# chayanchatterjee/GW-Whisper

Measured on AMD Instinct MI355X. Metric: 1s-strain segments/sec (encoder fwd), higher is better.
Workload: dtype bf16; 1 GPU; whisper-tiny encoder fwd, batch 256 log-mel (80x3000) per GPU, 1500 tokens, random-init weights (BASELINE configs[1]); global_batch=256, parallelism=dp1, encoder=tiny, streams_per_gpu=1

## Files before the change

### gw_whisper_amd/csrc/mlp_fused.hip

```cpp
#include "common.h"

#include <stdlib.h>

#include <type_traits>

namespace gww {

namespace {
constexpr int MF_D = 384;
constexpr int MF_KT = MF_D / 64;
constexpr int MF_OT = MF_D / 32;
constexpr int MF_WAVES = 4, MF_THREADS = 256, MF_BM = 128;
#ifndef GWW_MF_EXP
#define GWW_MF_EXP 0
#endif
#ifndef GWW_MF_ABL
#define GWW_MF_ABL 0
#endif
#ifndef GWW_MF_OLDDMA
#define GWW_MF_OLDDMA 0
#endif
#ifndef GWW_MF_AHEAD
#define GWW_MF_AHEAD 3
#endif
// ... 13 lines not shown
#define MF_NT " nt"
#else
#define MF_NT ""
#endif
#ifndef GWW_MF_PADNOP
#define GWW_MF_PADNOP 0
#endif
#if GWW_MF_PADNOP
#define MF_PADNOP "s_nop 1\n\t"
#else
#define MF_PADNOP ""
#endif
#ifndef GWW_MF_XLDS
#define GWW_MF_XLDS 0
#endif
#ifndef GWW_MF_XSTNT
#define GWW_MF_XSTNT 0
#endif
#ifndef GWW_MF_XNT
#define GWW_MF_XNT 0
#endif
#if GWW_MF_XNT
#define MF_XNT MF_NT
#else
#define MF_XNT ""
#endif
#ifndef GWW_MF_XN_LDNT
#define GWW_MF_XN_LDNT 1
#endif
#ifndef GWW_MF_XN_STNT
#define GWW_MF_XN_STNT 1
#endif
#if GWW_MF_XN_LDNT
#define MF_XN_LDNT " nt"
#else
#define MF_XN_LDNT ""
#endif
#if GWW_MF_XN_STNT
#define MF_XN_STNT " nt"
#else
#define MF_XN_STNT ""
#endif
#ifndef GWW_MF_DMAGAP
#define GWW_MF_DMAGAP 1
#endif
#ifndef GWW_MF_TAIL2
#define GWW_MF_TAIL2 0
#endif
#ifndef GWW_MF_NORM
#define GWW_MF_NORM 1
#endif
#ifndef GWW_MF_XACC
#define GWW_MF_XACC 1
#endif
constexpr int MF_AHEAD = GWW_MF_AHEAD;
constexpr int MF_NST_MAX = MF_AHEAD + 1;
constexpr int MF_TILE = 128 * 64 * 2;
constexpr int MF_GL = 16 / MF_WAVES;
constexpr int MF_FMAX = 1536;
constexpr int MF_SLICE_STRIDE = 144, MF_SLICE_BYTES = 32 * MF_SLICE_STRIDE;
constexpr int MF_OFF_CB = MF_NST_MAX * MF_TILE;
constexpr int MF_OFF_U = MF_OFF_CB + MF_FMAX * 4;
constexpr int MF_OFF_B2 = MF_OFF_U + MF_FMAX * 4;
constexpr int MF_OFF_BO = MF_OFF_B2 + MF_D * 4;
constexpr int MF_OFF_QCB = MF_OFF_BO + MF_D * 4;
constexpr int MF_OFF_SLICE = MF_OFF_QCB + MF_FMAX * 4;
constexpr int MF_LDS = MF_OFF_SLICE + 2 * MF_WAVES * MF_SLICE_BYTES;
static_assert(MF_LDS <= 160 * 1024, "LDS budget");

template <int N>
using MF_FL = std::integral_constant<int, N>;

__device__ __forceinline__ float mf_sum8(float v) {
  v += __builtin_bit_cast(float, __builtin_amdgcn_update_dpp(0, __builtin_bit_cast(int, v), 0xB1, 0xF, 0xF, true));
  v += __builtin_bit_cast(float, __builtin_amdgcn_update_dpp(0, __builtin_bit_cast(int, v), 0x4E, 0xF, 0xF, true));
  v += __builtin_bit_cast(float, __builtin_amdgcn_update_dpp(0, __builtin_bit_cast(int, v), 0x141, 0xF, 0xF, true));
  return v;
}

template <int N>
__device__ __forceinline__ void mf_wait_vmcnt() {
  asm volatile("s_waitcnt vmcnt(%0)" ::"n"(N) : "memory");
}

__device__ __forceinline__ float gelu_sig(float x) {
  const float s = fminf(x * x, 64.0f);
  float q = fmaf(s, 0.0010148164f, -0.1067791331f);
  q = fmaf(s, q, -2.3011178f);
#if GWW_MF_EXP & 32
  const float e = (x * q) * 0.37f;
  return x * ((1.0f + e) * 0.91f);
#else
  const float e = __builtin_amdgcn_exp2f(x * q);
  return x * __builtin_amdgcn_rcpf(1.0f + e);
#endif
}

#ifdef GWW_STAMP
__device__ unsigned long long g_stamp_mlp[24];
#define MSTAMP_DECL unsigned long long _t0 = __builtin_amdgcn_s_memtime(); unsigned long long _acc[20] = {0}; \
  const unsigned long long _tb = _t0, _rb = __builtin_amdgcn_s_memrealtime();
#define MSTAMP(i)                                                  \
  do {                                                             \
    if (GWW_STAMP >= 2 && (i) != 0 && (i) != 3 && (i) != 4 && (i) != 5 && !((i) >= 100)) break; \
    __builtin_amdgcn_sched_barrier(0);                             \
    const unsigned long long _t1 = __builtin_amdgcn_s_memtime();   \
    _acc[(i) >= 100 ? (i) - 100 : (i)] += _t1 - _t0;               \
    _t0 = _t1;                                                     \
    __builtin_amdgcn_sched_barrier(0);                             \
  } while (0)
#define TSTAMP(i) do { if (GWW_STAMP == 3) MSTAMP(100 + (i)); } while (0)
#define MSTAMP_FLUSH                                                                 \
  if (lane == 0) {                                                                   \
    for (int _q = 0; _q < 20; ++_q) atomicAdd(&g_stamp_mlp[_q], _acc[_q]);           \
    atomicAdd(&g_stamp_mlp[21], __builtin_amdgcn_s_memrealtime() - _rb);             \
    atomicAdd(&g_stamp_mlp[22], __builtin_amdgcn_s_memtime() - _tb);                 \
    atomicAdd(&g_stamp_mlp[23], 1ull);                                                \
  }
#else
#define MSTAMP_DECL
#define MSTAMP(i)
#define TSTAMP(i)
#define MSTAMP_FLUSH
#endif
}

__device__ __forceinline__ const float* mf_x0_row(const MfX0& z, const float* X, long g, bool x0, bool& tail, int& seg) {
  tail = false; seg = 0;
  if (!x0) return X + g * MF_D;
  const unsigned b = (unsigned)g / (unsigned)z.T, j = (unsigned)g - b * (unsigned)z.T;
  seg = (int)b;
  tail = (int)j >= z.Tt - 2 && (int)j <= z.T - 2;
  if (tail) return z.pos + (long)j * MF_D;
  return z.xs + ((long)b * z.Tt + ((int)j == z.T - 1 ? z.Tt - 1 : (int)j)) * MF_D;
}

struct MfNoX0 {};
template <int MODE, bool OP, bool X0 = false, int XL = 0>
__global__ __launch_bounds__(MF_THREADS, 1) void k_mlp_fused(const float* X, const unsigned short* delta, float* x_out,
                                                            const float* __restrict__ ln_u,
                                                            const float* __restrict__ ln_cb,
                                                            const unsigned short* __restrict__ Wt,
                                                            const float* __restrict__ b2,
                                                            unsigned short* __restrict__ C, long M, int F,
                                                            int stagger_ticks, const float* __restrict__ q_u,
                                                            const float* __restrict__ q_cb,
                                                            unsigned short* __restrict__ q_out, int NQ,
                                                            float* x_next, const float* __restrict__ bo, int keep_x_new,
                                                            const std::conditional_t<X0, MfX0, MfNoX0> z) {
  __shared__ __attribute__((aligned(16))) unsigned char lds[MF_LDS];
  constexpr bool QKV = MODE == 1 || MODE == 2, LNQ = MODE == 2, FIN = MODE == 3;
  static_assert(!X0 || (GWW_MF_NORM && GWW_MF_XACC && (MODE == 2 || (MODE == 1 && OP))), "X0: layer 0's two launches; stages in the u table");
  constexpr bool XACC = GWW_MF_XACC && GWW_MF_NORM && GWW_MF_SCHED && OP && (MODE == 1 || MODE == 3);
  constexpr bool XIN = (XL & 1) != 0, XOUT = (XL & 2) != 0;
  static_assert(XL == 0 || (XACC && !GWW_MF_XLDS && !X0 && (!XOUT || MODE == 1) && XL <= 3), "XL: the accumulator-order stream of XACC");
  constexpr int MF_NST = MF_AHEAD + 1;
  float* lds_cb = reinterpret_cast<float*>(lds + MF_OFF_CB);
  float* lds_u = reinterpret_cast<float*>(lds + MF_OFF_U);
  float* lds_b2 = reinterpret_cast<float*>(lds + MF_OFF_B2);
  float* lds_bo = reinterpret_cast<float*>(lds + MF_OFF_BO);
  float* lds_qcb = reinterpret_cast<float*>(lds + MF_OFF_QCB);
  constexpr int OP_TILES = OP ? 3 * MF_KT : 0;
  typedef __attribute__((address_space(3))) void* lds_ptr;

  const int tid = threadIdx.x, lane = tid & 63, wave = tid >> 6;
  const int r = lane & 31, hh = lane >> 5;
  const long m_base = (long)blockIdx.x * MF_BM + wave * 32;
  unsigned char* slice = lds + MF_OFF_SLICE + wave * MF_SLICE_BYTES;
  unsigned char* const slice0 = slice;
  const int crow = lane >> 3, cchunk = lane & 7;

  const int wave_u = __builtin_amdgcn_readfirstlane(wave);
  const unsigned lane_off = (unsigned)lane * 16u;
  const unsigned lds_base = (unsigned)(unsigned long long)(lds_ptr)lds;
  auto issue_piece_c = [&](int tile, int stage, auto j_c) {
    constexpr int J = decltype(j_c)::value;
    const unsigned dst = lds_base + (unsigned)(stage * MF_TILE + MF_GL * wave_u * 1024);
    if (GWW_MF_EXP & 8) tile &= 7;
    const unsigned short* src = Wt + ((long)tile * (MF_TILE / 2) + MF_GL * wave_u * 512);
    const unsigned lo = lane_off;
    asm volatile("s_mov_b32 m0, %2\n\ts_nop 0\n\tglobal_load_lds_dwordx4 %0, %1 offset:%3"
                 :
                 : "v"(lo), "s"(src), "s"(dst), "n"(J * 1024)
                 : "memory");
  };
  auto issue_piece = [&](int tile, int stage, int j) {
#if GWW_MF_OLDDMA
    const unsigned dst = lds_base + (unsigned)(stage * MF_TILE + (MF_GL * wave_u + j) * 1024);
    const unsigned short* src = Wt + ((long)tile * (MF_TILE / 2) + (MF_GL * wave_u + j) * 512);
    unsigned keep;
    asm volatile("s_mov_b32 %0, m0\n\ts_mov_b32 m0, %3\n\ts_nop 0\n\tglobal_load_lds_dwordx4 %1, %2\n\ts_mov_b32 m0, %0"
                 : "=&s"(keep) : "v"(lane_off), "s"(src), "s"(dst) : "memory");
#else
    if (j == 0) issue_piece_c(tile, stage, std::integral_constant<int, 0>{});
    else if (j == 1) issue_piece_c(tile, stage, std::integral_constant<int, 1>{});
    else if (j == 2) issue_piece_c(tile, stage, std::integral_constant<int, 2>{});
    else issue_piece_c(tile, stage, std::integral_constant<int, 3>{});
#endif
  };
  auto issue = [&](int tile, int stage) {
#pragma unroll
    for (int j = 0; j < MF_GL; ++j) issue_piece(tile, stage, j);
  };

  MSTAMP_DECL
  auto stage_tables = [&]() {
    for (int i = tid; i < F; i += MF_THREADS) {
      lds_cb[i] = GWW_MF_SCHED ? ln_cb[i] * 0.125f : ln_cb[i];
      if (!GWW_MF_NORM) lds_u[i] = ln_u[i];
    }
    if (!GWW_MF_NORM && FIN) __syncthreads();
    if (!LNQ)
      for (int i = tid; i < MF_D; i += MF_THREADS) lds_b2[i] = XACC ? b2[i] + bo[i] : b2[i];
    if (OP)
      for (int i = tid; i < MF_D; i += MF_THREADS) lds_bo[i] = bo[i];
    if (FIN)
      for (int i = tid; i < MF_D; i += MF_THREADS) { lds_u[i] = q_u[i]; lds_u[MF_D + i] = q_cb[i]; }
    if (QKV && GWW_MF_NORM)
      for (int i = tid; i < NQ; i += MF_THREADS) lds_qcb[i] = q_cb[i];
  };
  if constexpr (!XACC) stage_tables();
  if (stagger_ticks > 0 && blockIdx.x < 256) {
    const unsigned long long t0 = __builtin_amdgcn_s_memrealtime();
    const unsigned long long wait = (unsigned long long)((blockIdx.x >> 3) & 15) * stagger_ticks;
    while (__builtin_amdgcn_s_memrealtime() - t0 < wait) __builtin_amdgcn_s_sleep(8);
  }

#pragma unroll
  for (int p = 0; p < MF_AHEAD; ++p) issue(p, p);
  const long xrow_l = m_base + r < M ? m_base + r : M - 1;
  const unsigned xoff = (unsigned)xrow_l * (unsigned)(MF_D * 4) + 16u * (unsigned)hh;
  const unsigned xoff_n = (unsigned)(xrow_l >> 5) * (unsigned)(32 * MF_D * 4) + 16u * (((unsigned)xrow_l & 31u) + 32u * (unsigned)hh);
  f32x4 xp[XACC ? MF_OT : 1][4];
  bool x0 = false;
  int x0_seg0 = 0;
  f32x4* const lds_x0 = reinterpret_cast<f32x4*>(lds + MF_OFF_U);
  const float* x0_stage[2] = {nullptr, nullptr};
  f32x4 x0_sg[2];
  bool x0_tail = false;
  int x0_seg = 0;
  if constexpr (X0) {
    x0 = __builtin_amdgcn_readfirstlane(*z.flag) != 0;
    const unsigned g0 = (unsigned)blockIdx.x * (unsigned)MF_BM;
    x0_seg0 = (int)(g0 / (unsigned)z.T);
    const int seg_last = (int)((unsigned)(M - 1) / (unsigned)z.T);
#pragma unroll
    for (int k = 0; k < 2; ++k) {
      const int q = tid + 256 * k < 4 * (MF_D / 4) ? tid + 256 * k : tid;
      const int sg = q / (2 * (MF_D / 4)), wh = (q / (MF_D / 4)) & 1, c = q % (MF_D / 4);
      const long b = x0_seg0 + sg < seg_last ? x0_seg0 + sg : seg_last;
      x0_stage[k] = (wh ? z.tr + b * MF_D : z.xs + (b * z.Tt + (z.Tt - 2)) * MF_D) + 4 * c;
    }
  }
  auto x0_publish = [&](f32x4 (&sg)[2]) {
    lds_x0[tid] = sg[0];
    if (tid + 256 < 4 * (MF_D / 4)) lds_x0[tid + 256] = sg[1];
    asm volatile("s_waitcnt lgkmcnt(0)" ::: "memory");
    __builtin_amdgcn_s_barrier();
    asm volatile("" ::: "memory");
  };
  if constexpr (XACC && X0) {
    const float* xsrc = mf_x0_row(z, X, xrow_l, x0, x0_tail, x0_seg) + 4 * hh;
#pragma unroll
    for (int t = 0; t < MF_OT; ++t)
#pragma unroll
      for (int cc = 0; cc < 4; ++cc)
        asm volatile("global_load_dwordx4 %0, %1, off offset:%2" MF_XNT : "=a"(xp[t][cc]) : "v"(xsrc), "n"((32 * t + 8 * cc) * 4) : "memory");
#pragma unroll
    for (int k = 0; k < 2; ++k) asm volatile("global_load_dwordx4 %0, %1, off" : "=v"(x0_sg[k]) : "v"(x0_stage[k]) : "memory");
  } else if constexpr (XACC) {
#pragma unroll
    for (int t = 0; t < MF_OT; ++t)
#pragma unroll
      for (int cc = 0; cc < 4; ++cc)
        if (GWW_MF_ABL & 32) asm volatile("v_accvgpr_write_b32 %0, 0" : "=a"(xp[t][cc][0]));
        else if constexpr (XIN)
          asm volatile("global_load_dwordx4 %0, %1, %2 offset:%3" MF_XN_LDNT : "=a"(xp[t][cc]) : "v"(xoff_n), "s"(reinterpret_cast<const char*>(X) + 4096 * t), "n"(1024 * cc) : "memory");
        else asm volatile("global_load_dwordx4 %0, %1, %2 offset:%3" MF_XNT : "=a"(xp[t][cc]) : "v"(xoff), "s"(X), "n"((32 * t + 8 * cc) * 4) : "memory");
  }
  bf16x8 af[MF_KT * 4];
  float row_rstd, row_mean;
  long grow[4];
#pragma unroll
  for (int i = 0; i < 4; ++i) {
    const long g = m_base + 8 * i + crow;
    grow[i] = g < M ? g : M - 1;
  }
  if constexpr (XACC) {
    const unsigned coff = (unsigned)xrow_l * (unsigned)(MF_D * 2) + 64u * (unsigned)hh;
#pragma unroll
    for (int S = 0; S < MF_KT; ++S)
#pragma unroll
      for (int j = 0; j < 4; ++j)
        asm volatile("global_load_dwordx4 %0, %1, %2 offset:%3" : "=v"(af[4 * S + j]) : "v"(coff), "s"(delta), "n"((64 * S + 8 * j) * 2) : "memory");
    if constexpr (X0) {
      if (x0) {
        asm volatile("s_waitcnt vmcnt(24)" : "+v"(x0_sg[0]), "+v"(x0_sg[1]) : : "memory");
#pragma unroll
        for (int t = 0; t < MF_OT; ++t) asm volatile("" : "+a"(xp[t][0]), "+a"(xp[t][1]), "+a"(xp[t][2]), "+a"(xp[t][3]));
        x0_publish(x0_sg);
        if (x0_tail) {
          const f32x4* const st = lds_x0 + (x0_seg - x0_seg0) * (2 * (MF_D / 4)) + hh;
#pragma unroll
          for (int t = 0; t < MF_OT; ++t)
#pragma unroll
            for (int cc = 0; cc < 4; ++cc) {
              const f32x4 xt = st[8 * t + 2 * cc], rt = st[MF_D / 4 + 8 * t + 2 * cc];
#pragma unroll
              for (int k = 0; k < 4; ++k) xp[t][cc][k] = __builtin_fmaf(xt[k], rt[k], xp[t][cc][k]);
            }
        }
      }
    }
    stage_tables();
    asm volatile("s_waitcnt vmcnt(0)" ::: "memory");
#pragma unroll
    for (int i = 0; i < MF_KT * 4; ++i) asm volatile("" : "+v"(af[i]));
    row_rstd = 1.f; row_mean = 0.f;
  } else if constexpr (OP) {
    const unsigned short* crow_p[4];
#pragma unroll
    for (int i = 0; i < 4; ++i) crow_p[i] = delta + grow[i] * MF_D + 8 * cchunk;
    u32x4 cv[MF_KT][4];
#pragma unroll
    for (int S = 0; S < MF_KT; ++S)
#pragma unroll
      for (int i = 0; i < 4; ++i) {
        if (GWW_MF_ABL & 64) { cv[S][i] = u32x4{0x3f803f80u, 0x3f803f80u, 0x3f803f80u, 0x3f803f80u}; continue; }
        asm volatile("global_load_dwordx4 %0, %1, off offset:%2" MF_NT : "=v"(cv[S][i]) : "v"(crow_p[i]), "n"(64 * S * 2) : "memory");
      }
#pragma unroll
    for (int S = 0; S < MF_KT; ++S) {
#pragma unroll
      for (int i = 0; i < 4; ++i) {
        if (!(GWW_MF_ABL & 64)) asm volatile("s_waitcnt vmcnt(%1)" : "+v"(cv[S][i]) : "n"(23 - (4 * S + i)));
        *reinterpret_cast<u32x4*>(slice + (8 * i + crow) * MF_SLICE_STRIDE + cchunk * 16) = cv[S][i];
      }
#pragma unroll
      for (int j = 0; j < 4; ++j) {
        u32x4 u = *reinterpret_cast<const u32x4*>(slice + r * MF_SLICE_STRIDE + (4 * hh + j) * 16);
        asm volatile("" : "+v"(u)::"memory");
        af[4 * S + j] = __builtin_bit_cast(bf16x8, u);
      }
    }
    row_rstd = 1.f; row_mean = 0.f;
  } else
  {
    float s1[4] = {0.f, 0.f, 0.f, 0.f}, s2[4] = {0.f, 0.f, 0.f, 0.f}, cshift[4];
    const float* xrow[4];
    const unsigned short* drow[4];
#pragma unroll
    for (int i = 0; i < 4; ++i) {
      xrow[i] = X + grow[i] * MF_D + 4 * cchunk;
      drow[i] = LNQ ? nullptr : delta + grow[i] * MF_D + 4 * cchunk;
    }
    bool tl[4] = {false, false, false, false};
    const f32x4* st_row[4] = {lds_x0, lds_x0, lds_x0, lds_x0};
    if constexpr (X0) {
#pragma unroll
      for (int i = 0; i < 4; ++i) {
        int seg;
        xrow[i] = mf_x0_row(z, X, grow[i], x0, tl[i], seg) + 4 * cchunk;
        st_row[i] = lds_x0 + (seg - x0_seg0) * (2 * (MF_D / 4)) + cchunk;
      }
#pragma unroll
      for (int k = 0; k < 2; ++k) asm volatile("global_load_dwordx4 %0, %1, off" : "=v"(x0_sg[k]) : "v"(x0_stage[k]) : "memory");
    }
#pragma unroll
    for (int S3 = 0; S3 < MF_KT; S3 += 3) {
      f32x4 xv[3][2][4];
// ... 63 lines not shown
        for (int j = 0; j < 4; ++j) {
          u32x4 u = *reinterpret_cast<const u32x4*>(slice + r * MF_SLICE_STRIDE + (4 * hh + j) * 16);
          asm volatile("" : "+v"(u)::"memory");
          af[4 * S + j] = __builtin_bit_cast(bf16x8, u);
        }
      }
    }
    TSTAMP(8);
    float* stat = reinterpret_cast<float*>(slice);
#pragma unroll
    for (int i = 0; i < 4; ++i) {
      float a = s1[i], b = s2[i];
      a = mf_sum8(a); b = mf_sum8(b);
      const float mean = a * (1.0f / MF_D);
      const float var = fmaxf(b * (1.0f / MF_D) - mean * mean, 0.f);
      if (cchunk == 0) {
        stat[8 * i + crow] = rsqrtf(var + 1e-5f);
        stat[32 + 8 * i + crow] = mean;
      }
    }
    row_rstd = stat[r];
    row_mean = stat[32 + r];
    asm volatile("" : "+v"(row_rstd), "+v"(row_mean)::"memory");
    TSTAMP(9);
  }
#if GWW_MF_NORM
  auto normalise_af = [&]() {
    const float nm = -row_mean * row_rstd;
#pragma unroll
    for (int i = 0; i < MF_KT * 4; ++i) {
      u32x4 w = __builtin_bit_cast(u32x4, af[i]);
#pragma unroll
      for (int q = 0; q < 4; ++q)
        w[q] = pack2bf(fmaf(bf2f((unsigned short)(w[q] & 0xffff)), row_rstd, nm), fmaf(bf2f((unsigned short)(w[q] >> 16)), row_rstd, nm));
      af[i] = __builtin_bit_cast(bf16x8, w);
    }
  };
  if (!OP) normalise_af();
#endif
  MSTAMP(0);

  int off1[8], off2[4];
#pragma unroll
  for (int j = 0; j < 8; ++j) off1[j] = r * 256 + ((((j >> 2) * 8 + 4 * hh + (j & 3)) ^ (r & 15)) << 4);
#pragma unroll
  for (int j = 0; j < 4; ++j) off2[j] = r * 128 + (((2 * j + hh) ^ ((r >> 1) & 7)) << 4);
  int offq[4];
#pragma unroll
  for (int j = 0; j < 4; ++j) offq[j] = r * 128 + (((4 * hh + j) ^ ((r >> 1) & 7)) << 4);

  f32x16 sacc[4], oacc[MF_OT];
  if constexpr (XACC) {
#pragma unroll
    for (int t = 0; t < MF_OT; ++t) {
      asm volatile("" : "+a"(xp[t][0]), "+a"(xp[t][1]), "+a"(xp[t][2]), "+a"(xp[t][3]));
      const auto lo = __builtin_shufflevector(xp[t][0], xp[t][1], 0, 1, 2, 3, 4, 5, 6, 7);
      const auto hi = __builtin_shufflevector(xp[t][2], xp[t][3], 0, 1, 2, 3, 4, 5, 6, 7);
      oacc[t] = __builtin_shufflevector(lo, hi, 0, 1, 2, 3, 4, 5, 6, 7, 8, 9, 10, 11, 12, 13, 14, 15);
    }
  } else {
#pragma unroll
    for (int t = 0; t < MF_OT; ++t)
#pragma unroll
      for (int j = 0; j < 16; ++j) oacc[t][j] = 0.f;
  }
  u32x4 pf[4][2];

  float a_u[2][4], a_b[2][4], a_v[2][4];
  auto act_begin = [&](int slot, int c, int p) {
    if (GWW_MF_EXP & 2) return;
    if (GWW_MF_SCHED) {
      a_b[slot][0] = a_b[slot][1] = a_b[slot][2] = a_b[slot][3] = 0.f;
      return;
    }
    const int nl = 128 * c + 32 * (p >> 2) + 8 * (p & 3) + 4 * hh;
#if !GWW_MF_NORM
    const float4 uv = *reinterpret_cast<const float4*>(lds_u + nl);
    a_u[slot][0] = uv.x; a_u[slot][1] = uv.y; a_u[slot][2] = uv.z; a_u[slot][3] = uv.w;
#endif
    if (GWW_MF_EXP & 16) {
      a_b[slot][0] = a_b[slot][1] = a_b[slot][2] = a_b[slot][3] = row_rstd;
      return;
    }
    const float4 bv = *reinterpret_cast<const float4*>(lds_cb + nl);
    a_b[slot][0] = bv.x; a_b[slot][1] = bv.y; a_b[slot][2] = bv.z; a_b[slot][3] = bv.w;
  };
  auto act_val = [&](int slot, int p, int e) {
    if (GWW_MF_EXP & 2) {
      a_v[slot][e] = sacc[p >> 2][4 * (p & 3) + e];
      return;
    }
#if GWW_MF_SCHED
    a_v[slot][e] = 0.125f * gelu_sig(8.0f * sacc[p >> 2][4 * (p & 3) + e]);
#elif GWW_MF_NORM
    a_v[slot][e] = gelu_sig(sacc[p >> 2][4 * (p & 3) + e] + a_b[slot][e]);
#else
    a_v[slot][e] = gelu_sig(fmaf(row_rstd, fmaf(-row_mean, a_u[slot][e], sacc[p >> 2][4 * (p & 3) + e]), a_b[slot][e]));
#endif
  };
  auto act_end = [&](int slot, int p) {
    const int t = p >> 2, cc = p & 3;
    pf[t][cc >> 1][2 * (cc & 1)] = pack2bf(a_v[slot][0], a_v[slot][1]);
    pf[t][cc >> 1][2 * (cc & 1) + 1] = pack2bf(a_v[slot][2], a_v[slot][3]);
    asm volatile("" : "+v"(pf[t][cc >> 1][2 * (cc & 1)]), "+v"(pf[t][cc >> 1][2 * (cc & 1) + 1]));
  };
  auto act_piece = [&](int slot, int c, int p) {
    act_begin(slot, c, p);
    act_val(slot, p, 0); act_val(slot, p, 1); act_val(slot, p, 2); act_val(slot, p, 3);
    act_end(slot, p);
  };

  float g_t[4] = {0.f, 0.f, 0.f, 0.f}, g_w[4] = {0.f, 0.f, 0.f, 0.f}, g_q[4] = {0.f, 0.f, 0.f, 0.f};
#define MF_FENCE()                                                                                                       \
  asm volatile("" : "+v"(g_t[0]), "+v"(g_t[1]), "+v"(g_t[2]), "+v"(g_t[3]), "+v"(g_w[0]), "+v"(g_w[1]), "+v"(g_w[2]),   \
               "+v"(g_w[3]), "+v"(g_q[0]), "+v"(g_q[1]), "+v"(g_q[2]), "+v"(g_q[3]))
  auto preload_bias = [&](int t, int chunk, int q) {
    const float4 bv = *reinterpret_cast<const float4*>(lds_cb + 64 * chunk + 32 * (t & 1) + 8 * q + 4 * hh);
    sacc[t][4 * q] = bv.x; sacc[t][4 * q + 1] = bv.y; sacc[t][4 * q + 2] = bv.z; sacc[t][4 * q + 3] = bv.w;
  };
  auto gelu_slice = [&](int t, int g) {
    if (GWW_MF_EXP & 2) return;
    const int k = g / 12, j = g % 12;
#pragma unroll
    for (int pr = 0; pr < 2; ++pr) {
      const int op = j - pr;
      if (op < 0 || op > 8) continue;
#pragma unroll
      for (int sl = 0; sl < 2; ++sl) {
        const int i = 2 * pr + sl, v = 4 * k + i;
        const float S_ = sacc[t][v];
        float& T_ = g_t[i];
        float& W_ = g_w[i];
        float& Q_ = g_q[i];
        if (op == 0) asm("v_mul_f32_e64 %0, %1, %1 clamp" : "=v"(W_) : "v"(S_));
        else if (op == 1) Q_ = fmaf(W_, 33.2535038f, -54.67091615f);
        else if (op == 2) Q_ = fmaf(W_, Q_, -18.4089424f);
        else if (op == 3) W_ = S_ * Q_;
        else if (op == 4) W_ = __builtin_amdgcn_exp2f(W_);
        else if (op == 5) W_ = 1.0f + W_;
        else if (op == 6) W_ = __builtin_amdgcn_rcpf(W_);
        else if (op == 7) T_ = S_ * W_;
        else if (op == 8 && sl == 1) {
          pf[t][k >> 1][2 * (k & 1) + pr] = pack2bf(g_t[2 * pr], g_t[2 * pr + 1]);
          asm volatile("" : "+v"(pf[t][k >> 1][2 * (k & 1) + pr]));
        }
      }
    }
  };

  TSTAMP(10);
  mf_wait_vmcnt<0>();
  __builtin_amdgcn_s_barrier();
  TSTAMP(11);

  bf16x8 wf[2][4];
  if (!LNQ && !OP) {
#pragma unroll
    for (int t = 0; t < 4; ++t)
      wf[0][t] = *reinterpret_cast<const bf16x8*>(lds + (t & 1) * 8192 + off1[t >> 1]);
  }
  if (OP) {
#pragma unroll
    for (int u = 0; u < 4; ++u) wf[0][u] = *reinterpret_cast<const bf16x8*>(lds + u * 4096 + offq[0]);
  }

  const int nck = F / 64;
  const int total = OP_TILES + 6 * nck + (QKV ? (NQ / 128) * MF_KT : 0);
  int stage = 0;
  int it = 0;

  auto first_off = [&](int kind, int u) -> int {
    return kind == 0 ? (u & 1) * 8192 + off1[u >> 1] : (kind == 1 ? u * 4096 + off2[0] : u * 4096 + offq[0]);
  };

  auto run_tile = [&](auto flat_c, auto kind_c, auto par_c, auto idx3_c, auto ride_t_c, int ride_cpair, int next_kind,
                      auto pre_c, int pre_chunk, auto pad_c) {
    constexpr int KIND = decltype(kind_c)::value, PAR = decltype(par_c)::value, IDX3 = decltype(idx3_c)::value;
    constexpr int RIDE_T = decltype(ride_t_c)::value;
    constexpr bool PAD = decltype(pad_c)::value != 0;
    constexpr bool NOWAIT = decltype(pad_c)::value == 2;
    constexpr int PRE = decltype(pre_c)::value;
    constexpr int ST = (12 % MF_NST == 0) ? ((decltype(flat_c)::value + OP_TILES) % MF_NST) : -1;
    if (ST >= 0) stage = ST;
    if constexpr (!(GWW_MF_EXP & 64)) {
      if (!NOWAIT) mf_wait_vmcnt<MF_GL * (MF_AHEAD - 2)>();
      __builtin_amdgcn_s_barrier();
    }
    MSTAMP(1);
    const int dma_tile = it + MF_AHEAD < total ? it + MF_AHEAD : total - 1;
    const int dma_stage = stage + MF_AHEAD >= MF_NST ? stage + MF_AHEAD - MF_NST : stage + MF_AHEAD;
    const int stage_next = stage + 1 == MF_NST ? 0 : stage + 1;
    MSTAMP(2);
#pragma unroll
    for (int sub = 0; sub < 4; ++sub) {
      bf16x8(&cur)[4] = wf[sub & 1];
      bf16x8(&nxt)[4] = wf[(sub + 1) & 1];
      const unsigned char* Wn = lds + (sub == 3 ? stage_next : stage) * MF_TILE;
      const int j12 = 4 * IDX3 + sub;
      const int v0 = (16 * j12) / 12, v1 = (16 * (j12 + 1)) / 12;
      __builtin_amdgcn_sched_barrier(0);
      constexpr bool DMA_IN_GAPS = GWW_MF_SCHED && GWW_MF_DMAGAP && RIDE_T >= 0;
      if (!(GWW_MF_EXP & 1) && !DMA_IN_GAPS) issue_piece(dma_tile, dma_stage, sub);
      if (!GWW_MF_SCHED && RIDE_T >= 0) {
#pragma unroll
// ... 203 lines not shown
            f32x4* const sp = reinterpret_cast<f32x4*>(reinterpret_cast<char*>(dst) + (XL != 0 && MODE == 1 ? xst_n : xoff) + (32 * t + 8 * cc) * 4);
            if (GWW_MF_XSTNT) __builtin_nontemporal_store(v, sp);
            else *sp = v;
          }
        }
        if (GWW_MF_XLDS && dst && !(GWW_MF_ABL & 16) && cc == 3) {
#pragma unroll
          for (int i = 0; i < 4; ++i) {
            const f32x4 u = *reinterpret_cast<const f32x4*>(slice0 + (t & 1) * (MF_WAVES * MF_SLICE_BYTES) + (8 * i + crow) * MF_SLICE_STRIDE + cchunk * 16);
            *reinterpret_cast<f32x4*>(reinterpret_cast<char*>(dst) + (unsigned)grow[i] * (unsigned)(MF_D * 4) + 16u * (unsigned)cchunk + t * 128) = u;
          }
        }
        if (t == 0 && cc == 0) {
          const auto sw = __builtin_amdgcn_permlane32_swap(__float_as_uint(v[0]), __float_as_uint(v[0]), false, false);
          csh = hh ? __uint_as_float(sw[0]) : v[0];
        }
        v[0] -= csh; v[1] -= csh; v[2] -= csh; v[3] -= csh;
        s1 += (v[0] + v[1]) + (v[2] + v[3]);
        s2 += (v[0] * v[0] + v[1] * v[1]) + (v[2] * v[2] + v[3] * v[3]);
      }
    {
      const auto a = __builtin_amdgcn_permlane32_swap(__float_as_uint(s1), __float_as_uint(s1), false, false);
      const auto b = __builtin_amdgcn_permlane32_swap(__float_as_uint(s2), __float_as_uint(s2), false, false);
      s1 = __uint_as_float(a[0]) + __uint_as_float(a[1]);
      s2 = __uint_as_float(b[0]) + __uint_as_float(b[1]);
    }
    const float mean_s = s1 * (1.0f / MF_D);
    row_rstd = rsqrtf(fmaxf(s2 * (1.0f / MF_D) - mean_s * mean_s, 0.f) + 1e-5f);
    row_mean = csh + mean_s;
    const float nm = -mean_s * row_rstd;
    asm volatile("" : "+a"(oacc[0]), "+a"(oacc[1]), "+a"(oacc[2]), "+a"(oacc[3]), "+a"(oacc[4]), "+a"(oacc[5]), "+a"(oacc[6]),
                      "+a"(oacc[7]), "+a"(oacc[8]), "+a"(oacc[9]), "+a"(oacc[10]), "+a"(oacc[11]));
#pragma unroll
    for (int S = 0; S < MF_KT; ++S)
#pragma unroll
      for (int cc = 0; cc < 4; ++cc) {
        const float4 be = *reinterpret_cast<const float4*>(sb + 64 * S + 8 * cc + 4 * hh);
        const float4 bo_ = *reinterpret_cast<const float4*>(sb + 64 * S + 32 + 8 * cc + 4 * hh);
        const f32x16& E = oacc[2 * S];
        const f32x16& O = oacc[2 * S + 1];
        const unsigned e0 = pack2bf(fmaf(E[4 * cc] + be.x - csh, row_rstd, nm), fmaf(E[4 * cc + 1] + be.y - csh, row_rstd, nm));
        const unsigned e1 = pack2bf(fmaf(E[4 * cc + 2] + be.z - csh, row_rstd, nm), fmaf(E[4 * cc + 3] + be.w - csh, row_rstd, nm));
        const unsigned o0 = pack2bf(fmaf(O[4 * cc] + bo_.x - csh, row_rstd, nm), fmaf(O[4 * cc + 1] + bo_.y - csh, row_rstd, nm));
        const unsigned o1 = pack2bf(fmaf(O[4 * cc + 2] + bo_.z - csh, row_rstd, nm), fmaf(O[4 * cc + 3] + bo_.w - csh, row_rstd, nm));
        const auto w0 = __builtin_amdgcn_permlane32_swap(e0, o0, false, false);
        const auto w1 = __builtin_amdgcn_permlane32_swap(e1, o1, false, false);
        const u32x4 f = {w0[0], w1[0], w0[1], w1[1]};
        af[4 * S + cc] = __builtin_bit_cast(bf16x8, f);
      }
      }
  };
  if constexpr (OP) {
    static_assert(12 % MF_NST == 0, "OP mode relies on a ring whose depth divides the 12-tile body (4 or 6 stages)");
#pragma unroll
    for (int nt = 0; nt < 3; ++nt) {
#pragma unroll
      for (int kt = 0; kt < MF_KT; ++kt) {
        const int itile = nt * MF_KT + kt;
        if (!(GWW_MF_ABL & 128)) mf_wait_vmcnt<MF_GL * (MF_AHEAD - 2)>();
        __builtin_amdgcn_s_barrier();
        const int st = itile % MF_NST, st_next = (itile + 1) % MF_NST, dma_st = (itile + MF_AHEAD) % MF_NST;
        const int dma_tile = itile + MF_AHEAD < total ? itile + MF_AHEAD : total - 1;
        const bool last = itile == OP_TILES - 1;
#pragma unroll
        for (int sub = 0; sub < 4; ++sub) {
          const int q = 4 * kt + sub;
          bf16x8(&cur)[4] = wf[q & 1];
          bf16x8(&nxt)[4] = wf[(q + 1) & 1];
          const unsigned char* Wn = lds + (sub == 3 ? st_next : st) * MF_TILE;
          if (!(GWW_MF_ABL & 128)) issue_piece(dma_tile, dma_st, sub);
#pragma unroll
          for (int u = 0; u < 4; ++u) {
            asm volatile(MF_PADNOP "v_mfma_f32_32x32x16_bf16 %0, %1, %2, %0" : "+a"(oacc[4 * nt + u]) : "v"(cur[u]), "v"(af[4 * kt + sub]));
            const int off = (last && sub == 3) ? (u & 1) * 8192 + off1[u >> 1] : u * 4096 + offq[(sub + 1) & 3];
            nxt[u] = *reinterpret_cast<const bf16x8*>(Wn + off);
          }
        }
      }
    }
    it = OP_TILES;
    stage = OP_TILES % MF_NST;
    TSTAMP(14);
    asm volatile("s_nop 15\n\ts_nop 15"
                 : "+a"(oacc[0]), "+a"(oacc[1]), "+a"(oacc[2]), "+a"(oacc[3]), "+a"(oacc[4]), "+a"(oacc[5]), "+a"(oacc[6]),
                   "+a"(oacc[7]), "+a"(oacc[8]), "+a"(oacc[9]), "+a"(oacc[10]), "+a"(oacc[11]));
    if constexpr (XACC) {
      if constexpr (XL != 0 && MODE == 1) {
        unsigned lo = lane_off;
        asm volatile("" : "+v"(lo));
        const long g = m_base + (long)((lo >> 4) & 31u);
        const unsigned gc = (unsigned)(g < M ? g : M - 1);
        seam_x(lds_bo, (keep_x_new && !(GWW_MF_ABL & 256)) ? x_out : nullptr, std::false_type{}, gc * (unsigned)(MF_D * 4) + ((lo >> 9) << 4));
      } else
      seam_x(lds_bo, (keep_x_new && !(GWW_MF_ABL & 256)) ? x_out : nullptr, std::false_type{}, 0u);
    } else {
    seam(X, x_out, lds_bo, [] {});
#if GWW_MF_NORM
    normalise_af();
#endif
#pragma unroll
    for (int t = 0; t < MF_OT; ++t)
#pragma unroll
      for (int j = 0; j < 16; ++j) oacc[t][j] = 0.f;
    }
    TSTAMP(15);
  }
  if constexpr (!LNQ) {
  if (GWW_MF_SCHED) {
#pragma unroll
    for (int t = 0; t < 4; ++t)
#pragma unroll
      for (int q = 0; q < 4; ++q) preload_bias(t, t >> 1, q);
  }
  using IW = std::conditional_t<OP && !XACC && !(GWW_MF_ABL & 32), I2, I1>;
  run_tile(MF_FL<0>{}, I0{}, I0{}, I0{}, IM{}, 0, 0, IM{}, 0, IW{});
  run_tile(MF_FL<1>{}, I0{}, I0{}, I1{}, IM{}, 0, 0, IM{}, 0, IW{});
  run_tile(MF_FL<2>{}, I0{}, I0{}, I2{}, IM{}, 0, 0, IM{}, 0, I1{});
  TSTAMP(12);
  if (GWW_MF_SCHED) asm volatile("s_nop 15\n\ts_nop 15" : "+v"(sacc[0]), "+v"(sacc[1]), "+v"(sacc[2]), "+v"(sacc[3]));
  act_piece(0, 0, 0); act_piece(0, 0, 1); act_piece(0, 0, 2); act_piece(0, 0, 3);
  TSTAMP(13);
  int b = 0;
  for (; b + 2 < nck; b += 2) {
// ... 468 lines not shown
#else
            const float4 bv = *reinterpret_cast<const float4*>(lds_qcb + nl);
            const float4 uv = *reinterpret_cast<const float4*>(lds_u + nl);
            const float v0 = fmaf(row_rstd, fmaf(-row_mean, uv.x, acc[t][4 * cc]), bv.x);
            const float v1 = fmaf(row_rstd, fmaf(-row_mean, uv.y, acc[t][4 * cc + 1]), bv.y);
            const float v2 = fmaf(row_rstd, fmaf(-row_mean, uv.z, acc[t][4 * cc + 2]), bv.z);
            const float v3 = fmaf(row_rstd, fmaf(-row_mean, uv.w, acc[t][4 * cc + 3]), bv.w);
#endif
            u32x2 o = {pack2bf(v0, v1), pack2bf(v2, v3)};
            *reinterpret_cast<u32x2*>(slice + r * MF_SLICE_STRIDE + (32 * tt + 8 * cc + 4 * hh) * 2) = o;
          }
        }
#pragma unroll
        for (int i = 0; i < 4; ++i) {
          const u32x4 u = *reinterpret_cast<const u32x4*>(slice + (8 * i + crow) * MF_SLICE_STRIDE + cchunk * 16);
          const long orow = m_base + 8 * i + crow;
          if (GWW_MF_ABL & 1) { asm volatile("" :: "v"(u)); continue; }
#if GWW_MF_NTSTORE
          __builtin_nontemporal_store(u, reinterpret_cast<u32x4*>(q_out + orow * NQ + nt * 128 + 64 * half + 8 * cchunk));
#else
          *reinterpret_cast<u32x4*>(q_out + orow * NQ + nt * 128 + 64 * half + 8 * cchunk) = u;
#endif
        }
      }
    }
    mf_wait_vmcnt<(GWW_MF_ABL & 3) ? 0 : 8>();
#endif
  }
  MSTAMP(3);
  MSTAMP_FLUSH
}

__device__ __forceinline__ u32x4 mf_scale_bf16x8(u32x4 v, float f) {
#pragma unroll
  for (int j = 0; j < 4; ++j) {
    const float lo = __uint_as_float(v[j] << 16) * f, hi = __uint_as_float(v[j] & 0xffff0000u) * f;
    v[j] = (__float_as_uint(lo) >> 16) | (__float_as_uint(hi) & 0xffff0000u);
  }
  return v;
}

__global__ __launch_bounds__(256) void k_mlp_pack(const unsigned short* __restrict__ w1,
                                                  const unsigned short* __restrict__ w2,
                                                  const unsigned short* __restrict__ wq,
                                                  unsigned short* __restrict__ out, int F, long n_chunks16,
                                                  const unsigned short* __restrict__ wo) {
  const int nck = F / 64, mlp_tiles = 6 * nck, op_tiles = wo ? 3 * MF_KT : 0;
  for (long g = (long)blockIdx.x * 256 + threadIdx.x; g < n_chunks16; g += (long)gridDim.x * 256) {
    const int tile_all = (int)(g >> 10), within = (int)(g & 1023);
    const int row = within >> 3, chunk = (within & 7) ^ ((row >> 1) & 7);
    const int tile = tile_all - op_tiles;
    u32x4 v;
    if (tile < 0) {
      const int nt = tile_all / MF_KT, kt = tile_all - nt * MF_KT;
      v = *reinterpret_cast<const u32x4*>(wo + (long)(128 * nt + row) * MF_D + 64 * kt + 8 * chunk);
    } else if (tile >= mlp_tiles) {
#if GWW_MF_TAIL2
      const int it2 = tile - mlp_tiles, cq = it2 / 3, k3 = it2 - 3 * cq;
      const int row2 = within >> 4, ch = (within & 15) ^ (row2 & 15);
      v = *reinterpret_cast<const u32x4*>(wq + (long)(64 * cq + row2) * MF_D + 128 * k3 + 8 * ch);
#else
      const int it2 = tile - mlp_tiles, nt = it2 / MF_KT, kt = it2 - nt * MF_KT;
      v = *reinterpret_cast<const u32x4*>(wq + (long)(128 * nt + row) * MF_D + 64 * kt + 8 * chunk);
#endif
    } else {
      int kind, cp, idx3;
      if (tile < 3) { kind = 0; cp = 0; idx3 = tile; }
      else {
        const int k = tile - 3, blk = k / 6, w = k - 6 * blk;
        if (blk == nck - 1) { kind = 1; cp = blk; idx3 = w; }
        else if (w < 3) { kind = 0; cp = blk + 1; idx3 = w; }
        else { kind = 1; cp = blk; idx3 = w - 3; }
      }
      if (kind == 0) {
        const int row2 = within >> 4, ch = (within & 15) ^ (row2 & 15);
        v = *reinterpret_cast<const u32x4*>(w1 + (long)(64 * cp + row2) * MF_D + 128 * idx3 + 8 * ch);
        if (GWW_MF_SCHED) v = mf_scale_bf16x8(v, 0.125f);
      } else {
        const unsigned short* src = w2 + (long)(128 * idx3 + row) * F + 64 * cp;
        unsigned short e[8];
#pragma unroll
        for (int j = 0; j < 8; ++j) {
          const int p = 8 * chunk + j;
          e[j] = src[(p & ~12) | ((p & 4) << 1) | ((p & 8) >> 1)];
        }
        v = u32x4{(unsigned)e[0] | ((unsigned)e[1] << 16), (unsigned)e[2] | ((unsigned)e[3] << 16),
                  (unsigned)e[4] | ((unsigned)e[5] << 16), (unsigned)e[6] | ((unsigned)e[7] << 16)};
        if (GWW_MF_SCHED) v = mf_scale_bf16x8(v, 8.0f);
      }
    }
    reinterpret_cast<u32x4*>(out)[g] = v;
  }
}

int launch_mlp_pack(const void* w1_folded, const void* w2, const void* wqkv_folded, void* out, int d, int F, int NQ,
                    hipStream_t s, const void* wo) {
  GWW_REQUIRE(d == MF_D && F % 128 == 0 && F >= 0 && (F > 0 || wqkv_folded),
              "mlp_pack: d must be 384 and ffn a multiple of 128 (0: only the q / k / v panel, for LayerNorm 1 + q / k / v alone)");
  GWW_REQUIRE(!wqkv_folded || (NQ > 0 && NQ % 128 == 0), "mlp_pack: the q / k / v panel needs NQ %% 128 == 0");
  GWW_REQUIRE(!wo || F > 0, "mlp_pack: an out_proj panel goes in front of an MLP stream");
  const long n16 = ((wo ? (long)MF_D * MF_D : 0) + 2L * MF_D * F + (wqkv_folded ? (long)NQ * MF_D : 0)) / 8;
  hipLaunchKernelGGL(k_mlp_pack, dim3((unsigned)cdiv(n16, 256)), dim3(256), 0, s, (const unsigned short*)w1_folded,
                     (const unsigned short*)w2, (const unsigned short*)wqkv_folded, (unsigned short*)out, F, n16,
                     (const unsigned short*)wo);
  GWW_LAUNCH_CHECK();
  return GWW_OK;
}
// ... 174 lines not shown
```

Measured before the change: 25970 segments/s.

## Spread delta and residual loads across the out-projection prologue loop

Under XACC, the fused out-projection+MLP kernel now issues only the first K-slice of the attention-context (delta) operand up front. The remaining slices ride along inside the out-projection MFMA loop, which is reordered to kt-outer/nt-inner, and the weight pack kernel is changed to match that tile order. Residual X tiles 4..11 and the LN/bias tables are loaded into registers and published to LDS later, after the prologue wait, instead of being staged from global memory before the loop. This shortens the exposed startup latency before the first MFMA, at the cost of hand-derived vmcnt counts that are tied to a 3-ahead, 4-piece ring.

```diff
diff --git a/gw_whisper_amd/csrc/mlp_fused.hip b/gw_whisper_amd/csrc/mlp_fused.hip
--- a/gw_whisper_amd/csrc/mlp_fused.hip
+++ b/gw_whisper_amd/csrc/mlp_fused.hip
@@ -89,6 +89,9 @@
 #endif
 #ifndef GWW_MF_XACC
 #define GWW_MF_XACC 1
+#endif
+#ifndef GWW_MF_CSPREAD
+#define GWW_MF_CSPREAD 1
 #endif
 constexpr int MF_AHEAD = GWW_MF_AHEAD;
 constexpr int MF_NST_MAX = MF_AHEAD + 1;
@@ -190,6 +193,8 @@
   static_assert(!X0 || (GWW_MF_NORM && GWW_MF_XACC && (MODE == 2 || (MODE == 1 && OP))), "X0: layer 0's two launches; stages in the u table");
   constexpr bool XACC = GWW_MF_XACC && GWW_MF_NORM && GWW_MF_SCHED && OP && (MODE == 1 || MODE == 3);
   constexpr bool XIN = (XL & 1) != 0, XOUT = (XL & 2) != 0;
+  constexpr bool CSP = GWW_MF_CSPREAD && XACC;
+  constexpr bool XPR = CSP && !X0 && !(GWW_MF_ABL & 32);
   static_assert(XL == 0 || (XACC && !GWW_MF_XLDS && !X0 && (!XOUT || MODE == 1) && XL <= 3), "XL: the accumulator-order stream of XACC");
   constexpr int MF_NST = MF_AHEAD + 1;
   float* lds_cb = reinterpret_cast<float*>(lds + MF_OFF_CB);
@@ -257,6 +262,55 @@
       for (int i = tid; i < NQ; i += MF_THREADS) lds_qcb[i] = q_cb[i];
   };
   if constexpr (!XACC) stage_tables();
+  constexpr int TB_CB = MF_FMAX / MF_THREADS, TB_D = (MF_D + MF_THREADS - 1) / MF_THREADS;
+  float tb_cb[TB_CB], tb_b2[TB_D], tb_bo[TB_D], tb_q[QKV ? TB_CB : TB_D], tb_qu[TB_D];
+  auto table_piece = [&](float& v, const float* p, int i, int n) {
+    const unsigned off = 4u * (unsigned)(i < n ? i : n - 1);
+    asm volatile("global_load_dword %0, %1, %2" : "=v"(v) : "v"(off), "s"(p) : "memory");
+  };
+  auto request_tables = [&]() {
+#pragma unroll
+    for (int k = 0; k < TB_CB; ++k) table_piece(tb_cb[k], ln_cb, tid + MF_THREADS * k, F);
+#pragma unroll
+    for (int k = 0; k < TB_D; ++k) { table_piece(tb_b2[k], b2, tid + MF_THREADS * k, MF_D); table_piece(tb_bo[k], bo, tid + MF_THREADS * k, MF_D); }
+    if constexpr (FIN) {
+#pragma unroll
+      for (int k = 0; k < TB_D; ++k) { table_piece(tb_qu[k], q_u, tid + MF_THREADS * k, MF_D); table_piece(tb_q[k], q_cb, tid + MF_THREADS * k, MF_D); }
+    }
+    if constexpr (QKV) {
+#pragma unroll
+      for (int k = 0; k < TB_CB; ++k) table_piece(tb_q[k], q_cb, tid + MF_THREADS * k, NQ);
+    }
+  };
+  auto publish_tables = [&]() {
+#pragma unroll
+    for (int k = 0; k < TB_CB; ++k) {
+      asm volatile("" : "+v"(tb_cb[k]));
+      if (tid + MF_THREADS * k < F) lds_cb[tid + MF_THREADS * k] = tb_cb[k] * 0.125f;
+    }
+#pragma unroll
+    for (int k = 0; k < TB_D; ++k) {
+      asm volatile("" : "+v"(tb_b2[k]), "+v"(tb_bo[k]));
+      if (tid + MF_THREADS * k < MF_D) {
+        lds_b2[tid + MF_THREADS * k] = tb_b2[k] + tb_bo[k];
+        lds_bo[tid + MF_THREADS * k] = tb_bo[k];
+      }
+    }
+    if constexpr (FIN) {
+#pragma unroll
+      for (int k = 0; k < TB_D; ++k) {
+        asm volatile("" : "+v"(tb_qu[k]), "+v"(tb_q[k]));
+        if (tid + MF_THREADS * k < MF_D) { lds_u[tid + MF_THREADS * k] = tb_qu[k]; lds_u[MF_D + tid + MF_THREADS * k] = tb_q[k]; }
+      }
+    }
+    if constexpr (QKV) {
+#pragma unroll
+      for (int k = 0; k < TB_CB; ++k) {
+        asm volatile("" : "+v"(tb_q[k]));
+        if (tid + MF_THREADS * k < NQ) lds_qcb[tid + MF_THREADS * k] = tb_q[k];
+      }
+    }
+  };
   if (stagger_ticks > 0 && blockIdx.x < 256) {
     const unsigned long long t0 = __builtin_amdgcn_s_memrealtime();
     const unsigned long long wait = (unsigned long long)((blockIdx.x >> 3) & 15) * stagger_ticks;
@@ -265,9 +319,11 @@
 
 #pragma unroll
   for (int p = 0; p < MF_AHEAD; ++p) issue(p, p);
+  if constexpr (XACC) request_tables();
   const long xrow_l = m_base + r < M ? m_base + r : M - 1;
   const unsigned xoff = (unsigned)xrow_l * (unsigned)(MF_D * 4) + 16u * (unsigned)hh;
   const unsigned xoff_n = (unsigned)(xrow_l >> 5) * (unsigned)(32 * MF_D * 4) + 16u * (((unsigned)xrow_l & 31u) + 32u * (unsigned)hh);
+  const unsigned coff = (unsigned)xrow_l * (unsigned)(MF_D * 2) + 64u * (unsigned)hh;
   f32x4 xp[XACC ? MF_OT : 1][4];
   bool x0 = false;
   int x0_seg0 = 0;
@@ -307,7 +363,7 @@
     for (int k = 0; k < 2; ++k) asm volatile("global_load_dwordx4 %0, %1, off" : "=v"(x0_sg[k]) : "v"(x0_stage[k]) : "memory");
   } else if constexpr (XACC) {
 #pragma unroll
-    for (int t = 0; t < MF_OT; ++t)
+    for (int t = 0; t < (XPR ? 4 : MF_OT); ++t)
 #pragma unroll
       for (int cc = 0; cc < 4; ++cc)
         if (GWW_MF_ABL & 32) asm volatile("v_accvgpr_write_b32 %0, 0" : "=a"(xp[t][cc][0]));
@@ -324,15 +380,23 @@
     grow[i] = g < M ? g : M - 1;
   }
   if constexpr (XACC) {
-    const unsigned coff = (unsigned)xrow_l * (unsigned)(MF_D * 2) + 64u * (unsigned)hh;
-#pragma unroll
-    for (int S = 0; S < MF_KT; ++S)
+#pragma unroll
+    for (int S = 0; S < (CSP ? 1 : MF_KT); ++S)
 #pragma unroll
       for (int j = 0; j < 4; ++j)
         asm volatile("global_load_dwordx4 %0, %1, %2 offset:%3" : "=v"(af[4 * S + j]) : "v"(coff), "s"(delta), "n"((64 * S + 8 * j) * 2) : "memory");
+    if constexpr (XPR) {
+#pragma unroll
+      for (int t = 4; t < MF_OT; ++t)
+#pragma unroll
+        for (int cc = 0; cc < 4; ++cc)
+          if constexpr (XIN)
+            asm volatile("global_load_dwordx4 %0, %1, %2 offset:%3" MF_XN_LDNT : "=a"(xp[t][cc]) : "v"(xoff_n), "s"(reinterpret_cast<const char*>(X) + 4096 * t), "n"(1024 * cc) : "memory");
+          else asm volatile("global_load_dwordx4 %0, %1, %2 offset:%3" MF_XNT : "=a"(xp[t][cc]) : "v"(xoff), "s"(X), "n"((32 * t + 8 * cc) * 4) : "memory");
+    }
     if constexpr (X0) {
       if (x0) {
-        asm volatile("s_waitcnt vmcnt(24)" : "+v"(x0_sg[0]), "+v"(x0_sg[1]) : : "memory");
+        asm volatile("s_waitcnt vmcnt(%2)" : "+v"(x0_sg[0]), "+v"(x0_sg[1]) : "n"(CSP ? 4 : 4 * MF_KT) : "memory");
 #pragma unroll
         for (int t = 0; t < MF_OT; ++t) asm volatile("" : "+a"(xp[t][0]), "+a"(xp[t][1]), "+a"(xp[t][2]), "+a"(xp[t][3]));
         x0_publish(x0_sg);
@@ -349,10 +413,10 @@
         }
       }
     }
-    stage_tables();
-    asm volatile("s_waitcnt vmcnt(0)" ::: "memory");
-#pragma unroll
-    for (int i = 0; i < MF_KT * 4; ++i) asm volatile("" : "+v"(af[i]));
+    asm volatile("s_waitcnt vmcnt(%0)" ::"n"(XPR ? 32 : 0) : "memory");
+#pragma unroll
+    for (int i = 0; i < (CSP ? 4 : MF_KT * 4); ++i) asm volatile("" : "+v"(af[i]));
+    publish_tables();
     row_rstd = 1.f; row_mean = 0.f;
   } else if constexpr (OP) {
     const unsigned short* crow_p[4];
@@ -522,7 +586,7 @@
   f32x16 sacc[4], oacc[MF_OT];
   if constexpr (XACC) {
 #pragma unroll
-    for (int t = 0; t < MF_OT; ++t) {
+    for (int t = 0; t < (XPR ? 4 : MF_OT); ++t) {
       asm volatile("" : "+a"(xp[t][0]), "+a"(xp[t][1]), "+a"(xp[t][2]), "+a"(xp[t][3]));
       const auto lo = __builtin_shufflevector(xp[t][0], xp[t][1], 0, 1, 2, 3, 4, 5, 6, 7);
       const auto hi = __builtin_shufflevector(xp[t][2], xp[t][3], 0, 1, 2, 3, 4, 5, 6, 7);
@@ -619,7 +683,7 @@
   };
 
   TSTAMP(10);
-  mf_wait_vmcnt<0>();
+  mf_wait_vmcnt<XPR ? 32 : 0>();
   __builtin_amdgcn_s_barrier();
   TSTAMP(11);
 
@@ -929,12 +993,27 @@
   };
   if constexpr (OP) {
     static_assert(12 % MF_NST == 0, "OP mode relies on a ring whose depth divides the 12-tile body (4 or 6 stages)");
-#pragma unroll
-    for (int nt = 0; nt < 3; ++nt) {
-#pragma unroll
-      for (int kt = 0; kt < MF_KT; ++kt) {
-        const int itile = nt * MF_KT + kt;
-        if (!(GWW_MF_ABL & 128)) mf_wait_vmcnt<MF_GL * (MF_AHEAD - 2)>();
+    static_assert(!CSP || (MF_AHEAD == 3 && MF_GL == 4), "CSP: the riders' schedule is derived for a four-stage ring of four pieces per wave");
+#pragma unroll
+    for (int kt = 0; kt < MF_KT; ++kt) {
+#pragma unroll
+      for (int nt = 0; nt < 3; ++nt) {
+        const int itile = kt * 3 + nt;
+        const int rid_prev = !CSP || itile < 1 || itile > 13 ? 0 : itile == 1 ? 4 : (itile - 2) % 3 == 2 ? 2 : 1;
+        const int ring_wait = XPR && itile == 0 ? 32 : XPR && itile == 1 ? 16 + MF_GL + 4 : MF_GL * (MF_AHEAD - 2) + rid_prev + (CSP && itile == 2 ? 1 : 0);
+        if (!(GWW_MF_ABL & 128)) asm volatile("s_waitcnt vmcnt(%0)" ::"n"(ring_wait) : "memory");
+        if constexpr (XPR) {
+          if (kt == 0 && nt > 0) {
+#pragma unroll
+            for (int t = 4 * nt; t < 4 * nt + 4; ++t) {
+              asm volatile("" : "+a"(xp[t][0]), "+a"(xp[t][1]), "+a"(xp[t][2]), "+a"(xp[t][3]));
+              const auto lo = __builtin_shufflevector(xp[t][0], xp[t][1], 0, 1, 2, 3, 4, 5, 6, 7);
+              const auto hi = __builtin_shufflevector(xp[t][2], xp[t][3], 0, 1, 2, 3, 4, 5, 6, 7);
+              oacc[t] = __builtin_shufflevector(lo, hi, 0, 1, 2, 3, 4, 5, 6, 7, 8, 9, 10, 11, 12, 13, 14, 15);
+            }
+          }
+        }
+        if (CSP && nt == 0 && kt > 0) asm volatile("" : "+v"(af[4 * kt]), "+v"(af[4 * kt + 1]), "+v"(af[4 * kt + 2]), "+v"(af[4 * kt + 3]));
         __builtin_amdgcn_s_barrier();
         const int st = itile % MF_NST, st_next = (itile + 1) % MF_NST, dma_st = (itile + MF_AHEAD) % MF_NST;
         const int dma_tile = itile + MF_AHEAD < total ? itile + MF_AHEAD : total - 1;
@@ -946,6 +1025,12 @@
           bf16x8(&nxt)[4] = wf[(q + 1) & 1];
           const unsigned char* Wn = lds + (sub == 3 ? st_next : st) * MF_TILE;
           if (!(GWW_MF_ABL & 128)) issue_piece(dma_tile, dma_st, sub);
+          if constexpr (CSP) {
+            const int rm = (itile + 2) % 3, rS = (itile + 5) / 3;
+            const int cp = itile == 0 ? 4 + sub : itile > 12 ? -1 : sub == 1 ? 4 * rS + rm : sub == 2 && rm == 2 ? 4 * rS + 3 : -1;
+            if (cp >= 0)
+              asm volatile("global_load_dwordx4 %0, %1, %2 offset:%3" : "=v"(af[cp >= 0 ? cp : 0]) : "v"(coff), "s"(delta), "n"((64 * (cp / 4) + 8 * (cp % 4)) * 2) : "memory");
+          }
 #pragma unroll
           for (int u = 0; u < 4; ++u) {
             asm volatile(MF_PADNOP "v_mfma_f32_32x32x16_bf16 %0, %1, %2, %0" : "+a"(oacc[4 * nt + u]) : "v"(cur[u]), "v"(af[4 * kt + sub]));
@@ -1520,7 +1605,7 @@
     const int tile = tile_all - op_tiles;
     u32x4 v;
     if (tile < 0) {
-      const int nt = tile_all / MF_KT, kt = tile_all - nt * MF_KT;
+      const int kt = tile_all / 3, nt = tile_all - 3 * kt;
       v = *reinterpret_cast<const u32x4*>(wo + (long)(128 * nt + row) * MF_D + 64 * kt + 8 * chunk);
     } else if (tile >= mlp_tiles) {
 #if GWW_MF_TAIL2
```

Measured after the change: 26270 segments/s (median of 6 runs). 1.01x the previous value.
